# ntc-ai/sliders-conceptmod

Hardware: AMD Instinct MI355X
Metric: slider train-steps/sec (4-pass UNet fwd+bwd) (higher is better)
Workload: dtype fp16; 1 GPU; sdxl_1024_b2_r4; unet=sdxl, resolution=1024, per_gpu_batch=2, unet_batch=4, global_batch=2, lora_rank=4, train_method=noxattn, network_type=lierla, lora_params=2662400, scheduler=euler_a, parallelism=dp1, pre_roll=excluded, skip_dead_cfg_half=False, dedup_uncond=False, guidance_passes=1 batched UNet call (3 frozen + 1 adapted sub-batches)

## Files before the change

sliders_conceptmod_amd/csrc/gemm.hip:

```cpp
#include <cstdio>
#include <cstdlib>
#include <cstring>
#include <unordered_map>

#include "gemm_epilogue.h"
#include "gemm_tile.h"

#include <mutex>

namespace smi {

namespace {

constexpr int BM = 128, BN = 128, BK = 64;

struct ConvRow {
  int base;
  int oy, ox;
};

template <typename T, bool CONV>
__global__ __launch_bounds__(256) void gemm_nt_kernel(GemmParams p) {
  __shared__ __attribute__((aligned(16))) unsigned char smem[2 * BM * BK * 2];
  unsigned char* As = smem;
  unsigned char* Bs = smem + BM * BK * 2;

  const int tid = threadIdx.x;
  const int lane = tid & 63;
  const int wave = tid >> 6;
  const int wm = wave >> 1, wn = wave & 1;

  const int nbn = (p.N + BN - 1) / BN;
  const int wg = xcd_remap(blockIdx.x, gridDim.x);
  const int bm0 = (wg / nbn) * BM;
  const int bn0 = (wg % nbn) * BN;

  const uint32_t esz = 2;
  __amdgpu_buffer_rsrc_t rA, rW;
  if (CONV) {
    rA = make_rsrc(p.A, (uint32_t)((int64_t)p.Nb * p.Hin * p.Win * p.Cin * esz));
  } else {
    rA = make_rsrc(p.A, (uint32_t)(((int64_t)(p.M - 1) * p.lda + p.K) * esz));
  }
  rW = make_rsrc(p.W, (uint32_t)((int64_t)p.N * p.K * esz));

  const int sc = tid & 7;
  const int sr = tid >> 3;
  ConvRow crow[4];
  uint32_t a_rowoff[4];
  uint32_t w_rowoff[4];
#pragma unroll
  for (int i = 0; i < 4; ++i) {
    const int m = bm0 + sr + 32 * i;
    if (CONV) {
      if (m < p.M) {
        const int hw = p.Hout * p.Wout;
        const int img = m / hw;
        const int rem = m - img * hw;
        crow[i].base = img * p.Hin * p.Win;
        crow[i].oy = rem / p.Wout;
        crow[i].ox = rem - crow[i].oy * p.Wout;
      } else {
        crow[i].base = 0;
        crow[i].oy = -(1 << 20);
        crow[i].ox = -(1 << 20);
      }
      a_rowoff[i] = 0;
    } else {
      a_rowoff[i] = (m < p.M) ? (uint32_t)((int64_t)m * p.lda * esz) : OOB;
    }
    const int n = bn0 + sr + 32 * i;
    w_rowoff[i] = (n < p.N) ? (uint32_t)((int64_t)n * p.K * esz) : OOB;
  }

  u32x4 ra[4], rb[4];
  auto load_tile = [&](int kt) {
    const int k0 = kt * BK;
    const int kc = k0 + sc * 8;
    const bool kok = kc < p.K;
    if (CONV) {
      const int tap = k0 / p.Cin;
      const int c0 = k0 - tap * p.Cin;
      int ky, kx;
      conv_tap_yx(p, tap, ky, kx);
#pragma unroll
      for (int i = 0; i < 4; ++i) {
        int iy, ix;
        bool ok;
        if (p.transposed) {
          const int ty = crow[i].oy + 1 - ky, tx = crow[i].ox + 1 - kx;
          iy = ty / p.stride;
          ix = tx / p.stride;
          ok = (ty >= 0) && (tx >= 0) && (iy * p.stride == ty) && (ix * p.stride == tx) && (iy < p.Hin) &&
               (ix < p.Win);
        } else {
          iy = crow[i].oy * p.stride + ky + p.tap_oy;
          ix = crow[i].ox * p.stride + kx + p.tap_ox;
          if (p.upsample) {
            ok = (iy >= 0) && (ix >= 0) && (iy < 2 * p.Hin) && (ix < 2 * p.Win);
            iy >>= 1;
            ix >>= 1;
          } else {
            ok = (iy >= 0) && (ix >= 0) && (iy < p.Hin) && (ix < p.Win);
          }
        }
        const uint32_t off = ok ? (uint32_t)(((crow[i].base + iy * p.Win + ix) * (int64_t)p.Cin + c0 + sc * 8) * esz)
                                : OOB;
        ra[i] = buf_load16(rA, off);
      }
    } else {
#pragma unroll
      for (int i = 0; i < 4; ++i) {
        const uint32_t off = (kok && a_rowoff[i] != OOB) ? a_rowoff[i] + (uint32_t)kc * esz : OOB;
        ra[i] = buf_load16(rA, off);
      }
    }
#pragma unroll
    for (int i = 0; i < 4; ++i) {
      const uint32_t off = (kok && w_rowoff[i] != OOB) ? w_rowoff[i] + (uint32_t)kc * esz : OOB;
      rb[i] = buf_load16(rW, off);
    }
  };
  auto store_tile = [&]() {
#pragma unroll
    for (int i = 0; i < 4; ++i) {
      const int r = sr + 32 * i;
      const int off = r * 128 + ((sc ^ (r & 7)) << 4);
      *reinterpret_cast<u32x4*>(As + off) = ra[i];
      *reinterpret_cast<u32x4*>(Bs + off) = rb[i];
    }
  };

  f32x4 acc[4][4];
#pragma unroll
  for (int a = 0; a < 4; ++a)
#pragma unroll
    for (int b = 0; b < 4; ++b) acc[a][b] = f32x4{0.f, 0.f, 0.f, 0.f};

  const int nk = (p.K + BK - 1) / BK;
  const int fr = lane & 15;
  const int fq = lane >> 4;

  load_tile(0);
  for (int kt = 0; kt < nk; ++kt) {
    store_tile();
    __syncthreads();
    if (kt + 1 < nk) load_tile(kt + 1);
#pragma unroll
    for (int kk = 0; kk < 2; ++kk) {
      typename TT<T>::v8 xa[4], wb[4];
      const int ch = kk * 4 + fq;
#pragma unroll
      for (int i = 0; i < 4; ++i) {
        const int rm = wm * 64 + i * 16 + fr;
        Pack8<T> t;
        t.u = *reinterpret_cast<const u32x4*>(As + rm * 128 + ((ch ^ (rm & 7)) << 4));
        xa[i] = t.v;
        const int rn = wn * 64 + i * 16 + fr;
        Pack8<T> s;
        s.u = *reinterpret_cast<const u32x4*>(Bs + rn * 128 + ((ch ^ (rn & 7)) << 4));
        wb[i] = s.v;
      }
#pragma unroll
      for (int ni = 0; ni < 4; ++ni)
#pragma unroll
        for (int mi = 0; mi < 4; ++mi) acc[ni][mi] = TT<T>::mfma16(wb[ni], xa[mi], acc[ni][mi]);
    }
    __syncthreads();
  }

#pragma unroll
  for (int mi = 0; mi < 4; ++mi) {
    const int m = bm0 + wm * 64 + mi * 16 + fr;
    if (m >= p.M) continue;
    const bool lora_on = p.lora_r > 0 && m >= p.lora_row0;
    const int64_t vrow = p.rowvec ? epi_rowvec_offset(p, m) : 0;
#pragma unroll
    for (int ni = 0; ni < 4; ++ni) {
      const int n = bn0 + wn * 64 + ni * 16 + fq * 4;
      if (n >= p.N) continue;
      float v[4] = {acc[ni][mi][0], acc[ni][mi][1], acc[ni][mi][2], acc[ni][mi][3]};
      if (p.bias) epi_add<T, 4>(v, reinterpret_cast<const T*>(p.bias) + n);
      if (p.rowvec) epi_add<T, 4>(v, reinterpret_cast<const T*>(p.rowvec) + vrow + n);
      if (lora_on) epi_lora<4, false>(v, p, m, n);
      if (p.res) epi_add<T, 4>(v, reinterpret_cast<const T*>(p.res) + (int64_t)m * p.ldr + n);
      if (p.out_f32) epi_store_f32<4>(reinterpret_cast<float*>(p.C) + (int64_t)m * p.ldc + n, v);
      else epi_store<T, 4>(reinterpret_cast<T*>(p.C) + (int64_t)m * p.ldc + n, v);
    }
  }
}

template <typename T>
__global__ __launch_bounds__(256) void conv3x3_small_kernel(const T* __restrict__ in, const T* __restrict__ w,
                                                            const T* __restrict__ bias, void* out, int out_f32,
                                                            int Nb, int H, int W, int Cin, int Cout) {
  const int cg = (Cout + 3) / 4;
  const int64_t total = (int64_t)Nb * H * W * cg;
  for (int64_t idx = (int64_t)blockIdx.x * blockDim.x + threadIdx.x; idx < total;
       idx += (int64_t)gridDim.x * blockDim.x) {
    const int g = (int)(idx % cg);
    const int64_t pix = idx / cg;
    const int x = (int)(pix % W);
    const int y = (int)((pix / W) % H);
    const int n = (int)(pix / ((int64_t)W * H));
    const int co0 = g * 4;
    float acc[4] = {0.f, 0.f, 0.f, 0.f};
    for (int ky = 0; ky < 3; ++ky) {
      const int iy = y + ky - 1;
      if (iy < 0 || iy >= H) continue;
      for (int kx = 0; kx < 3; ++kx) {
        const int ix = x + kx - 1;
        if (ix < 0 || ix >= W) continue;
        const T* ip = in + (((int64_t)n * H + iy) * W + ix) * Cin;
        const int kb = (ky * 3 + kx) * Cin;
        for (int ci = 0; ci < Cin; ++ci) {
          const float v = to_f(ip[ci]);
#pragma unroll
          for (int j = 0; j < 4; ++j)
            if (co0 + j < Cout) acc[j] += v * to_f(w[(int64_t)(co0 + j) * 9 * Cin + kb + ci]);
        }
      }
    }
#pragma unroll
    for (int j = 0; j < 4; ++j) {
      if (co0 + j >= Cout) continue;
      float v = acc[j] + (bias ? to_f(bias[co0 + j]) : 0.f);
      if (out_f32)
        reinterpret_cast<float*>(out)[pix * Cout + co0 + j] = v;
      else
        reinterpret_cast<T*>(out)[pix * Cout + co0 + j] = from_f<T>(v);
    }
  }
}

template <typename T, int NS, int LR = 0>
__global__ __launch_bounds__(256) void splitk_finish_kernel(GemmParams p, const float* __restrict__ slab, int nsplit_rt) {
  const int nsplit = NS > 0 ? NS : nsplit_rt;
  const int n4 = p.N >> 2;
  const int64_t total = (int64_t)p.M * n4;
  const int64_t plane = (int64_t)p.M * p.N;
  for (int64_t idx = (int64_t)blockIdx.x * blockDim.x + threadIdx.x; idx < total; idx += (int64_t)gridDim.x * blockDim.x) {
    const int m = (int)(idx / n4);
    const int n = (int)(idx - (int64_t)m * n4) * 4;
    const float* sp = slab + (int64_t)m * p.N + n;
    f32x4 sum = *reinterpret_cast<const f32x4*>(sp);
    if constexpr (NS > 0) {
      f32x4 w[NS > 1 ? NS - 1 : 1];
#pragma unroll
      for (int s = 1; s < NS; ++s) w[s - 1] = *reinterpret_cast<const f32x4*>(sp + s * plane);
#pragma unroll
      for (int s = 1; s < NS; ++s)
#pragma unroll
        for (int j = 0; j < 4; ++j) sum[j] += w[s - 1][j];
    } else {
      for (int s = 1; s < nsplit; ++s) {
        const f32x4 w = *reinterpret_cast<const f32x4*>(sp + s * plane);
#pragma unroll
        for (int j = 0; j < 4; ++j) sum[j] += w[j];
      }
    }
    float v[4] = {sum[0], sum[1], sum[2], sum[3]};
    if (p.bias) epi_add<T, 4>(v, reinterpret_cast<const T*>(p.bias) + n);
    if (p.rowvec) epi_add<T, 4>(v, reinterpret_cast<const T*>(p.rowvec) + epi_rowvec_offset(p, m) + n);
    if (p.lora_r > 0 && m >= p.lora_row0) {
      if constexpr (LR > 0) epi_lora4_unrolled<LR>(v, p, m, n);
      else if (p.lora_r == 4) epi_lora4_unrolled<4>(v, p, m, n);
      else if (p.lora_r == 8) epi_lora4_unrolled<8>(v, p, m, n);
      else epi_lora<4, false>(v, p, m, n);
    }
    if (p.res) epi_add<T, 4>(v, reinterpret_cast<const T*>(p.res) + (int64_t)m * p.ldr + n);
    if (p.out_f32) epi_store_f32<4>(reinterpret_cast<float*>(p.C) + (int64_t)m * p.ldc + n, v);
    else epi_store<T, 4>(reinterpret_cast<T*>(p.C) + (int64_t)m * p.ldc + n, v);
  }
}

}

namespace {
struct TileName {
  GemmTile tile;
  const char* env;
  int code;
};
constexpr TileName kTileNames[] = {
    {GemmTile::Auto, nullptr, 0},
    {GemmTile::Auto, "no8ph", -1},
    {GemmTile::Auto, "no5ph", -1},
    {GemmTile::T128x128, nullptr, 13},
    {GemmTile::T128x128w8, "128", 1},
    {GemmTile::T128x128w8, nullptr, 5},
    {GemmTile::T256x128, "256", 2},
    {GemmTile::T64x128, "64", 14},
    {GemmTile::T64x128w4, "64w", 7},
    {GemmTile::T128x160, "160", 4},
    {GemmTile::T128x160w8, "160w", 10},
    {GemmTile::T128x160Deep, nullptr, 11},
    {GemmTile::T64x160, "64x160", 12},
    {GemmTile::Gemm3, "8ph", 100},
    {GemmTile::Gemm4, "5ph", 200},
    {GemmTile::V1, "v1", 300},
};
GemmTile tile_of_code(int code) {
  for (const TileName& t : kTileNames)
    if (t.code == code) return t.tile;
  return GemmTile::Auto;
}
int code_of_tile(GemmTile tile) {
  for (const TileName& t : kTileNames)
    if (t.tile == tile && t.code >= 0) return t.code;
  return 0;
}
const TileName* gemm_override() {
  static const TileName* o = []() -> const TileName* {
    const char* e = getenv("SMI_GEMM");
    for (const TileName& t : kTileNames)
      if (e && t.env && !strcmp(e, t.env)) return &t;
    return nullptr;
  }();
  return o;
}
bool forced_v1() { return gemm_override() && gemm_override()->tile == GemmTile::V1; }

GemmTile heuristic_tile(const GemmParams& p, bool gemm3) {
  if (gemm3 && !(p.conv && p.N % 256 != 0) && (int64_t)cdiv(p.M, 256) * cdiv(p.N, 256) >= 512 && gemm3_supported(p))
    return GemmTile::Gemm3;
  const bool rows256 = (int64_t)cdiv(p.M, 256) * cdiv(p.N, 128) >= 512 && (p.conv || p.N >= 4096);
  if (p.N % 160 == 0 && (!p.geglu_out || p.N % 320 == 0) && (int64_t)cdiv(p.M, 128) * cdiv(p.N, 128) >= 1024) {
    auto cost = [&](int bm, int bn, double eff) {
      const int64_t tiles = (int64_t)cdiv(p.M, bm) * cdiv(p.N, bn);
      return (double)((tiles + 255) / 256) * bm * bn / eff;
    };
    if (cost(128, 160, 1.04) < cost(rows256 ? 256 : 128, 128, rows256 ? 1.10 : 1.0)) return GemmTile::T128x160;
  }
  return rows256 ? GemmTile::T256x128 : GemmTile::T128x128w8;
}

GemmTile fit_tile(GemmTile tile, const GemmParams& p, bool gemm3) {
  switch (tile) {
    case GemmTile::Auto: return heuristic_tile(p, gemm3);
    case GemmTile::T64x128: return p.conv ? GemmTile::T128x128 : tile;
    case GemmTile::T128x160:
      return p.N % 8 == 0 && (!p.geglu_out || p.N % 320 == 0) ? tile : GemmTile::T128x128;
    case GemmTile::T64x160:
    case GemmTile::T128x160w8:
    case GemmTile::T128x160Deep: return p.N % 160 == 0 && !p.geglu_out ? tile : heuristic_tile(p, gemm3);
    case GemmTile::Gemm3: return gemm3_supported(p) ? tile : heuristic_tile(p, gemm3);
    case GemmTile::Gemm4: return gemm4_supported(p) ? tile : heuristic_tile(p, gemm3);
    default: return tile;
  }
}
int launch_tile(const GemmParams& p, GemmTile tile, hipStream_t stream) {
  if (tile == GemmTile::Gemm3) return launch_gemm3(p, stream);
  if (tile == GemmTile::Gemm4) return launch_gemm4(p, stream);
  if (tile == GemmTile::V1) return launch_v1(p, stream);
  return launch_gemm2(p, tile, stream);
}
}

bool gemm_geglu_supported(const GemmParams& p) { return !forced_v1() && gemm2_geglu_supported(p); }

namespace {
struct TuneKey {
  int v[18];
  bool operator==(const TuneKey& o) const { return memcmp(v, o.v, sizeof(v)) == 0; }
};
struct TuneHash {
  size_t operator()(const TuneKey& k) const {
    size_t h = 1469598103934665603ull;
    for (int x : k.v) h = (h ^ (size_t)(unsigned)x) * 1099511628211ull;
    return h;
  }
};
const char* tune_file() {
  static const char* f = getenv("SMI_TUNE_FILE");
  return (f && f[0]) ? f : nullptr;
}
std::unordered_map<TuneKey, int, TuneHash>& tune_cache() {
  static std::unordered_map<TuneKey, int, TuneHash> c;
  static bool loaded = false;
  if (!loaded) {
    loaded = true;
    if (const char* path = tune_file()) {
      if (FILE* fp = fopen(path, "r")) {
        for (;;) {
          TuneKey k;
          int choice = 0, got = 0;
          for (int i = 0; i < 18; ++i) got += fscanf(fp, "%d", &k.v[i]) == 1;
          got += fscanf(fp, "%d", &choice) == 1;
          if (got != 19) break;
          c[k] = choice;
        }
        fclose(fp);
      }
    }
  }
  return c;
}
void tune_persist(const TuneKey& k, int choice) {
  const char* path = tune_file();
  if (!path) return;
  if (FILE* fp = fopen(path, "a")) {
    for (int i = 0; i < 18; ++i) fprintf(fp, "%d ", k.v[i]);
    fprintf(fp, "%d\n", choice);
    fclose(fp);
  }
}
bool tune_enabled() {
  static int on = -1;
  if (on < 0) {
    const char* e = getenv("SMI_GEMM_TUNE");
    on = (e && !strcmp(e, "0")) ? 0 : 1;
  }
  return on == 1;
}
int launch_candidate(const GemmParams& p, GemmTile cand, hipStream_t stream) {
  return launch_tile(p, fit_tile(cand, p, true), stream);
}
GemmTile tuned_choice(const GemmParams& p, hipStream_t stream) {
  TuneKey key;
  const int taps = p.conv && (p.tap_w != 3 || p.tap_oy != -p.pad || p.tap_ox != -p.pad)
                       ? 16 * (p.tap_w * 64 + (p.tap_oy + 4) * 8 + (p.tap_ox + 4))
                       : 0;
  const int kv[18] = {(int)p.dtype, (int)p.conv, p.M, p.N, p.K, (int)(p.conv ? p.Cin : p.lda),
                      (int)(p.stride * 4 + p.upsample * 2 + p.transposed + taps), (int)(p.res != nullptr), p.lora_r,
                      (int)(p.geglu_out != nullptr), (int)p.out_f32, (int)(p.bias != nullptr),
                      (int)(p.rowvec != nullptr), (int)(p.conv ? p.Hin * 65536 + p.Win : p.ldc),
                      (int)(p.res ? p.ldr : 0), p.lora_seg, p.pad, (int)(p.res == p.C) + 2 * (int)(p.lora_r > 0 && p.up_sn == 1)};
  memcpy(key.v, kv, sizeof(kv));
  static std::mutex mu;
  std::lock_guard<std::mutex> lock(mu);
  auto& cache = tune_cache();
  auto it = cache.find(key);
  if (it != cache.end()) return tile_of_code(it->second);
  GemmTile cands[14];
  int nc = 0;
  cands[nc++] = GemmTile::Auto;
  const bool plain_conv = p.conv && p.stride == 1 && !p.upsample && !p.transposed;
  if (!p.conv || plain_conv) {
    cands[nc++] = GemmTile::T128x128w8;
    if ((int64_t)cdiv(p.M, 256) * cdiv(p.N, 128) >= 128) cands[nc++] = GemmTile::T256x128;
    if (p.N % 160 == 0 && (!p.geglu_out || p.N % 320 == 0)) cands[nc++] = GemmTile::T128x160;
    if (gemm3_supported(p) && (int64_t)cdiv(p.M, 256) * cdiv(p.N, 256) >= 192) cands[nc++] = GemmTile::Gemm3;
    if ((int64_t)cdiv(p.M, 128) * cdiv(p.N, 128) <= 512) cands[nc++] = GemmTile::T64x128w4;
    if (!p.geglu_out && p.N % 160 == 0 && (int64_t)cdiv(p.M, 128) * (p.N / 160) <= 256) cands[nc++] = GemmTile::T64x160;
    if (!p.geglu_out && p.N % 160 == 0 && p.K >= 1280 && (int64_t)cdiv(p.M, 128) * (p.N / 160) <= 128)
      cands[nc++] = GemmTile::T128x160Deep;
    if (gemm4_supported(p) && (int64_t)(p.M / 256) * (p.N / 320) >= 128) cands[nc++] = GemmTile::Gemm4;
    if (!p.geglu_out && p.N % 160 == 0 && p.N % 8 == 0 && (int64_t)cdiv(p.M, 128) * (p.N / 160) <= 512)
      cands[nc++] = GemmTile::T128x160w8;
  } else if (p.conv && p.upsample && gemm4_supported(p) && (int64_t)(p.M / 256) * (p.N / 320) >= 128) {
    cands[nc++] = GemmTile::Gemm4;
  }
  GemmTile best = GemmTile::Auto;
  if (nc > 1) {
    GemmParams q = p;
    void* tmp = nullptr;
    if (q.res == q.C) {
      const size_t bytes = ((size_t)(p.M - 1) * p.ldc + p.N) * (p.out_f32 ? 4 : 2);
      if (hipMalloc(&tmp, bytes) != hipSuccess) {
        (void)hipGetLastError();
        cache[key] = 0;
        return GemmTile::Auto;
      }
      q.C = tmp;
    }
    hipEvent_t a, b;
    if (hipEventCreate(&a) != hipSuccess || hipEventCreate(&b) != hipSuccess) {
      (void)hipGetLastError();
      if (tmp) (void)hipFree(tmp);
      cache[key] = 0;
      return GemmTile::Auto;
    }
    float tbest = 0.f, t0 = 0.f;
    static const bool dump = getenv("SMI_TUNE_DUMP") != nullptr;
    if (dump) fprintf(stderr, "[smi tune]");
    for (int i = 0; i < nc; ++i) {
      if (launch_candidate(q, cands[i], stream) != 0) continue;
      (void)hipEventRecord(a, stream);
      (void)launch_candidate(q, cands[i], stream);
      (void)launch_candidate(q, cands[i], stream);
      (void)hipEventRecord(b, stream);
      if (hipEventSynchronize(b) != hipSuccess) break;
      float ms = 0.f;
      (void)hipEventElapsedTime(&ms, a, b);
      if (dump) fprintf(stderr, " %d:%.1fus", code_of_tile(cands[i]), ms * 500.f);
      if (i == 0) { t0 = tbest = ms; continue; }
      if (ms < 0.97f * t0 && ms < tbest) { tbest = ms; best = cands[i]; }
    }
    if (dump)
      fprintf(stderr, "  -> %d   [%s M=%d N=%d K=%d%s%s%s%s]\n", code_of_tile(best), p.conv ? "conv" : "gemm", p.M, p.N, p.K,
              p.bias ? " bias" : "", p.res ? " res" : "", p.lora_r ? " lora" : "", p.geglu_out ? " geglu" : "");
    (void)hipEventDestroy(a);
    (void)hipEventDestroy(b);
    if (tmp) {
      (void)hipStreamSynchronize(stream);
      (void)hipFree(tmp);
    }
    (void)hipGetLastError();
  }
  cache[key] = code_of_tile(best);
  tune_persist(key, code_of_tile(best));
  return best;
}
}

namespace {
thread_local void* t_scratch = nullptr;
thread_local size_t t_scratch_bytes = 0;
int splitk_slices(const GemmParams& p) {
  static const bool on = []() { const char* e = getenv("SMI_GEMM_SPLITK"); return !(e && !strcmp(e, "0")); }();
  if (!on || !t_scratch || p.geglu_out || p.ksplit || !gemm2_supported(p) || p.N % 4 != 0) return 1;
  const int64_t tiles = (int64_t)cdiv(p.M, 128) * cdiv(p.N, 128);
  const int nk = cdiv(p.K, 64);
  static const int max_tiles = []() { const char* e = getenv("SMI_SPLITK_MAXTILES"); return e ? atoi(e) : 256; }();
  if (tiles > max_tiles || nk < 16) return 1;
  static const int few_tiles = []() { const char* e = getenv("SMI_SPLITK_FEWTILES"); return e ? atoi(e) : 95; }();
  static const int long_k = []() { const char* e = getenv("SMI_SPLITK_LONGK"); return e ? atoi(e) : 32; }();
  if (nk < long_k && tiles > few_tiles) return 1;
  int64_t lim = 16;
  const int64_t budget = 512;
  if (nk / 4 < lim) lim = nk / 4;
  const int64_t fit = (int64_t)(t_scratch_bytes / ((size_t)p.M * p.N * sizeof(float)));
  if (fit < lim) lim = fit;
  const int64_t tiles64 = (int64_t)cdiv(p.M, 64) * cdiv(p.N, 128);
  int64_t s = budget / tiles64 < lim ? budget / tiles64 : lim;
  if (s < 2) s = budget / tiles < lim ? budget / tiles : lim;
  return s < 1 ? 1 : (int)s;
}
int launch_splitk(const GemmParams& p, int S, GemmTile slice, hipStream_t stream) {
  SMI_CHECK(p.lora_seg % 4 == 0, "gemm: lora_seg %% 4 != 0");
  GemmParams q = p;
  q.C = t_scratch;
  q.ldc = p.N;
  q.out_f32 = 1;
  q.bias = q.res = q.rowvec = nullptr;
  q.lora_r = 0;
  q.lora_xa = q.lora_up = nullptr;
  q.ksplit = S;
  if (slice == GemmTile::Auto)
    slice = (int64_t)cdiv(p.M, 64) * cdiv(p.N, 128) * S <= 512 ? GemmTile::T64x128w4 : GemmTile::T128x128w8;
  if (launch_gemm2(q, slice, stream) != 0) return -1;
  const int64_t total = (int64_t)p.M * (p.N / 4);
  const int grid = (int)((total + 255) / 256 < 2048 ? (total + 255) / 256 : 2048);
#define FIN_R(TT_, NS_, LR_) hipLaunchKernelGGL((splitk_finish_kernel<TT_, NS_, LR_>), dim3(grid), dim3(256), 0, stream, p, (const float*)t_scratch, S)
#define FIN(TT_, NS_)                                                                                           \
  do {                                                                                                          \
    if (p.lora_r == 12) FIN_R(TT_, NS_, 12);                                                                    \
    else if (p.lora_r == 24) FIN_R(TT_, NS_, 24);                                                               \
    else FIN_R(TT_, NS_, 0);                                                                                    \
  } while (0)
#define FIN_T(TT_)                                                                                              \
  do {                                                                                                          \
    switch (S) {                                                                                                \
      case 2: FIN(TT_, 2); break;   case 3: FIN(TT_, 3); break;   case 4: FIN(TT_, 4); break;                   \
      case 5: FIN(TT_, 5); break;   case 6: FIN(TT_, 6); break;   case 7: FIN(TT_, 7); break;                   \
      case 8: FIN(TT_, 8); break;   case 9: FIN(TT_, 9); break;   case 10: FIN(TT_, 10); break;                 \
      case 11: FIN(TT_, 11); break; case 12: FIN(TT_, 12); break; case 13: FIN(TT_, 13); break;                 \
      case 14: FIN(TT_, 14); break; case 15: FIN(TT_, 15); break; case 16: FIN(TT_, 16); break;                 \
      default: FIN(TT_, 0);                                                                                     \
    }                                                                                                           \
  } while (0)
  if (p.dtype == DT_F16) FIN_T(f16); else FIN_T(bf16);
#undef FIN_T
#undef FIN
#undef FIN_R
  SMI_HIP(hipGetLastError());
  return 0;
}
}

namespace {
int g_upconv_phase_sel = -1;
}
void set_upconv_phase(int on) { g_upconv_phase_sel = on; }
bool upconv_phase_on() {
  static const bool env_on = []() { const char* e = getenv("SMI_UPCONV_PHASE"); return !(e && !strcmp(e, "0")); }();
  return g_upconv_phase_sel < 0 ? env_on : g_upconv_phase_sel != 0;
}
bool upconv_phase_takes(int lowres_pixels) {
  if (!upconv_phase_on()) return false;
  if (g_upconv_phase_sel > 0) return true;
  static const int floor_px = []() { const char* e = getenv("SMI_UPCONV_PHASE_MIN_PIXELS"); return e ? atoi(e) : 1024; }();
  return lowres_pixels >= floor_px;
}

void set_gemm_scratch(void* ws, size_t bytes) {
  t_scratch = ws;
  t_scratch_bytes = ws ? bytes : 0;
}

int launch_gemm(const GemmParams& p, hipStream_t stream) {
  SMI_CHECK(p.M > 0 && p.N > 0 && p.K > 0, "gemm: bad shape M=%d N=%d K=%d", p.M, p.N, p.K);
  SMI_CHECK(!p.geglu_out || gemm_geglu_supported(p), "gemm: fused GEGLU not available for this shape/layout");
  if (p.conv) {
    SMI_CHECK(p.K == p.tap_w * p.tap_w * p.Cin && p.M == p.Nb * p.Hout * p.Wout && (p.stride == 1 || p.stride == 2),
              "conv: inconsistent geometry");
    SMI_CHECK(p.tap_w == 3 || (p.tap_w == 2 && p.stride == 1 && !p.upsample && !p.transposed),
              "conv: a %d-wide tap grid (2 takes a plain stride-1 conv only)", p.tap_w);
  }
  static const bool splitk_debug = getenv("SMI_SPLITK_DEBUG") != nullptr;
  if (splitk_debug && gemm2_supported(p) && !p.geglu_out) {
    const char* es = getenv("SMI_SPLITK_S");
    const char* ev = getenv("SMI_SPLITK_V");
    const int S = es ? atoi(es) : 0;
    const GemmTile t = fit_tile(tile_of_code(ev ? atoi(ev) : 0), p, false);
    if (S > 1 && t_scratch && (size_t)S * p.M * p.N * sizeof(float) <= t_scratch_bytes) return launch_splitk(p, S, t, stream);
    if (S == 1) return launch_gemm2(p, t, stream);
  }
  const TileName* forced = gemm_override();
  if (!forced_v1()) {
    const int S = splitk_slices(p);
    if (S > 1) return launch_splitk(p, S, GemmTile::Auto, stream);
  }
  if (forced_v1() || !gemm2_supported(p)) return launch_v1(p, stream);
  if (forced) return launch_tile(p, fit_tile(forced->tile, p, false), stream);
  static int deep = -1, deep_k = 1280, small_grid = 128;
  if (deep < 0) {
    const char* e = getenv("SMI_GEMM_DEEP");
    deep = (e && !strcmp(e, "0")) ? 0 : 1;
    if (const char* k = getenv("SMI_GEMM_DEEP_K")) deep_k = atoi(k);
    if (const char* k = getenv("SMI_GEMM_SMALL_GRID")) small_grid = atoi(k);
  }
  const int64_t tiles160 = (int64_t)cdiv(p.M, 128) * (p.N / 160);
  if (deep && !p.geglu_out && p.N % 160 == 0 && p.K >= deep_k && tiles160 <= 320 && tiles160 > small_grid &&
      (!p.conv || (p.stride == 1 && !p.upsample && !p.transposed)))
    return launch_gemm2(p, GemmTile::T128x160Deep, stream);
  if (tune_enabled() && (int64_t)p.M * p.N >= (1 << 17)) return launch_candidate(p, tuned_choice(p, stream), stream);
  return launch_tile(p, heuristic_tile(p, true), stream);
}

int launch_gemm_on_tile(const GemmParams& p, int tile_code, int ksplit, int* ran_code, hipStream_t stream) {
  SMI_CHECK(p.M > 0 && p.N > 0 && p.K > 0, "gemm: bad shape M=%d N=%d K=%d", p.M, p.N, p.K);
  if (ran_code) *ran_code = 0;
  if (tile_code == 0 && ksplit <= 1) return launch_gemm(p, stream);
  GemmTile tile = tile_of_code(tile_code);
  SMI_CHECK(tile_code == 0 || tile != GemmTile::Auto, "gemm: unknown tile code %d", tile_code);
  SMI_CHECK(!p.geglu_out || gemm2_geglu_supported(p), "gemm: fused GEGLU not available for this shape/layout");
  tile = (tile == GemmTile::V1 || !gemm2_supported(p)) ? GemmTile::V1 : fit_tile(tile, p, false);
  if (ran_code) *ran_code = code_of_tile(tile);
  if (ksplit > 1) {
    SMI_CHECK(tile != GemmTile::V1 && tile != GemmTile::Gemm3 && tile != GemmTile::Gemm4 && !p.geglu_out && p.N % 4 == 0,
              "gemm: split-K takes a gemm2 tile as its slice kernel (tile code %d)", tile_code);
    SMI_CHECK(t_scratch && (size_t)ksplit * p.M * p.N * sizeof(float) <= t_scratch_bytes,
              "gemm: %d slices need a scratch of %zu bytes", ksplit, (size_t)ksplit * p.M * p.N * sizeof(float));
    return launch_splitk(p, ksplit, tile, stream);
  }
  return launch_tile(p, tile, stream);
}

int launch_v1(const GemmParams& p, hipStream_t stream) {
  SMI_CHECK(p.K % 8 == 0 && p.N % 4 == 0, "gemm: K %% 8 and N %% 4 must be 0 (K=%d N=%d)", p.K, p.N);
  SMI_CHECK(p.ldc % 4 == 0, "gemm: ldc %% 4 != 0");
  SMI_CHECK(p.lora_seg % 4 == 0, "gemm: lora_seg %% 4 != 0");
  SMI_CHECK(p.res == nullptr || p.ldr % 4 == 0, "gemm: ldr %% 4 != 0");
  if (p.conv) {
    SMI_CHECK(p.Cin % 64 == 0 && p.K == p.tap_w * p.tap_w * p.Cin, "conv: Cin %% 64 != 0 or K != taps*Cin (Cin=%d K=%d)",
              p.Cin, p.K);
    SMI_CHECK(p.M == p.Nb * p.Hout * p.Wout, "conv: M != Nb*Hout*Wout");
    SMI_CHECK((int64_t)p.Nb * p.Hin * p.Win * p.Cin * 2 < 0xFFFFFFF0ll, "conv: input larger than 4 GiB");
    SMI_CHECK(p.stride == 1 || p.stride == 2, "conv: stride");
  } else {
    SMI_CHECK(p.lda % 8 == 0, "gemm: lda %% 8 != 0");
    SMI_CHECK(((int64_t)(p.M - 1) * p.lda + p.K) * 2 < 0xFFFFFFF0ll, "gemm: A larger than 4 GiB");
  }
  SMI_CHECK((int64_t)p.N * p.K * 2 < 0xFFFFFFF0ll, "gemm: W larger than 4 GiB");
  const int grid = cdiv(p.M, BM) * cdiv(p.N, BN);
  if (p.dtype == DT_F16) {
    if (p.conv)
      hipLaunchKernelGGL((gemm_nt_kernel<f16, true>), dim3(grid), dim3(256), 0, stream, p);
    else
      hipLaunchKernelGGL((gemm_nt_kernel<f16, false>), dim3(grid), dim3(256), 0, stream, p);
  } else {
    if (p.conv)
      hipLaunchKernelGGL((gemm_nt_kernel<bf16, true>), dim3(grid), dim3(256), 0, stream, p);
    else
      hipLaunchKernelGGL((gemm_nt_kernel<bf16, false>), dim3(grid), dim3(256), 0, stream, p);
  }
  SMI_HIP(hipGetLastError());
  return 0;
}

int launch_conv3x3_small(int dtype, const void* in, const void* w, const void* bias, void* out, int out_f32, int Nb,
                         int H, int W, int Cin, int Cout, hipStream_t stream) {
  const int64_t total = (int64_t)Nb * H * W * ((Cout + 3) / 4);
  const int grid = (int)((total + 255) / 256 < 8192 ? (total + 255) / 256 : 8192);
  if (dtype == DT_F16)
    hipLaunchKernelGGL(conv3x3_small_kernel<f16>, dim3(grid), dim3(256), 0, stream, (const f16*)in, (const f16*)w,
                       (const f16*)bias, out, out_f32, Nb, H, W, Cin, Cout);
  else
    hipLaunchKernelGGL(conv3x3_small_kernel<bf16>, dim3(grid), dim3(256), 0, stream, (const bf16*)in,
                       (const bf16*)w, (const bf16*)bias, out, out_f32, Nb, H, W, Cin, Cout);
  SMI_HIP(hipGetLastError());
  return 0;
}

}
```

sliders_conceptmod_amd/csrc/gemm4.hip:

```cpp
#include "gemm_epilogue.h"
#include "gemm_tile.h"

namespace smi {
namespace {

constexpr int BM = 256, BN = 320, BK = 64;
constexpr int UNIT = 64 * BK * 2;
constexpr int ABYTES = 4 * UNIT;
constexpr int KBUF = ABYTES + 5 * UNIT;
constexpr int SMEM4 = 2 * KBUF;

template <typename T, int MODE>
__global__ __launch_bounds__(512) void gemm_5ph_kernel(GemmParams p) {
  constexpr bool CONV = MODE == 1 || MODE == 4;
  constexpr int TW = MODE == 4 ? 2 : 3;
  const int toy = MODE == 4 ? p.tap_oy : -1, tox = MODE == 4 ? p.tap_ox : -1;
  constexpr bool GEGLU = MODE == 2;
  constexpr bool UPS = MODE == 3;
  typedef typename TT<T>::v8 v8;
  extern __shared__ __attribute__((aligned(1024))) unsigned char smem[];

  const int tid = threadIdx.x;
  const int lane = tid & 63;
  const int wave = __builtin_amdgcn_readfirstlane(tid >> 6);
  const int wr = wave >> 1, wc = wave & 1, grp = wave >> 2;

  const int nbn = p.N / BN, nbm = p.M / BM;
  const int ntiles = nbn * nbm;
  const int nk = p.K / BK;
  const int G = gridDim.x;

  const int GW = raster_band(nbn);
  auto tile_origin = [&](int v, int& bm0, int& bn0) {
    int tm, tn;
    grouped_raster(xcd_remap(v, ntiles), nbm, nbn, GW, tm, tn);
    bm0 = __builtin_amdgcn_readfirstlane(tm * BM);
    bn0 = __builtin_amdgcn_readfirstlane(tn * BN);
  };

  const int lrow = lane >> 3, lslot = lane & 7;
  const int r64 = wave * 8 + lrow;
  const int chunk = lslot ^ lrow;
  const bool mix = !CONV && !UPS && p.lora_r > 0 && p.lora_row0 > 0 && 4 * (int64_t)p.lora_row0 == 3 * (int64_t)p.M;
  const int lda = (CONV || UPS) ? p.Cin : (int)p.lda;
  const bool arow = mix && wave >= 6;
  const uint32_t voffA = (uint32_t)(arow ? r64 - 48 : r64) * (uint32_t)(lda * 2) + chunk * 16;
  constexpr bool geglu = GEGLU;
  const int nhalf = p.N >> 1;
  const uint32_t voffB =
      (geglu ? (uint32_t)(((r64 >> 4) & 1) * nhalf + (r64 >> 5) * 80 + (r64 & 15))
             : (uint32_t)((r64 >> 5) * 160 + 8 * ((r64 & 15) >> 2) + 4 * ((r64 >> 4) & 1) + (r64 & 3))) *
          (uint32_t)(p.K * 2) +
      chunk * 16;
  const int64_t a_unit = (int64_t)(mix ? (arow ? 16 : 48) : 64) * lda * 2;
  const int64_t w_unit = (int64_t)(geglu ? 16 : 32) * p.K * 2;
  const int ldsw = wave * 1024;

  int bm0, bn0, bm1 = 0, bn1 = 0;
  int v = blockIdx.x;
  tile_origin(v, bm0, bn0);
  auto a_row0 = [&](int bm) { return mix ? (arow ? p.lora_row0 + (bm >> 2) : 3 * (bm >> 2)) : bm; };
  const char* a_cur = reinterpret_cast<const char*>(p.A) + (int64_t)a_row0(bm0) * lda * 2;
  const char* w_cur = reinterpret_cast<const char*>(p.W) + (int64_t)(geglu ? bn0 >> 1 : bn0) * p.K * 2;
  const char* a_nxt = a_cur;
  const char* w_nxt = w_cur;
  bool has_next = false;

  int am_cur[4] = {0, 0, 0, 0}, am_nxt[4] = {0, 0, 0, 0};
  auto conv_masks = [&](int bm, int (&am)[4]) {
    const int hw = p.Hin * p.Win;
#pragma unroll
    for (int u = 0; u < 4; ++u) {
      const int m = bm + u * 64 + r64;
      const int img = m / hw;
      const int rem = m - img * hw;
      const int oy = rem / p.Win, ox = rem - oy * p.Win;
      int mk = 0;
#pragma unroll
      for (int ky = 0; ky < TW; ++ky)
#pragma unroll
        for (int kx = 0; kx < TW; ++kx) {
          const bool ok = (unsigned)(oy + ky + toy) < (unsigned)p.Hin && (unsigned)(ox + kx + tox) < (unsigned)p.Win;
          mk |= ok ? (1 << (TW * ky + kx)) : 0;
        }
      am[u] = mk;
    }
  };
  if (CONV) conv_masks(bm0, am_cur);
  const int cpt = (CONV || UPS) ? p.Cin / BK : 1;
  const int cpt_magic = 65536 / cpt + 1;

  int ub_cur[4] = {0, 0, 0, 0}, uy_cur[4] = {0, 0, 0, 0}, ux_cur[4] = {0, 0, 0, 0};
  int ub_nxt[4] = {0, 0, 0, 0}, uy_nxt[4] = {0, 0, 0, 0}, ux_nxt[4] = {0, 0, 0, 0};
  auto ups_units = [&](int bm, int (&ub)[4], int (&uy)[4], int (&ux)[4]) {
    const int hw = p.Hout * p.Wout;
#pragma unroll
    for (int u = 0; u < 4; ++u) {
      const int m0 = bm + u * 64;
      const int img = m0 / hw;
      const int rem = m0 - img * hw;
      const int oy = rem / p.Wout;
      ub[u] = __builtin_amdgcn_readfirstlane(img * p.Hin * p.Win);
      uy[u] = __builtin_amdgcn_readfirstlane(oy);
      ux[u] = __builtin_amdgcn_readfirstlane(rem - oy * p.Wout);
    }
  };
  int voffU[3] = {0, 0, 0};
  if (UPS) {
    ups_units(bm0, ub_cur, uy_cur, ux_cur);
#pragma unroll
    for (int kx = 0; kx < 3; ++kx) voffU[kx] = ((r64 + kx - 1) >> 1) * (p.Cin * 2) + chunk * 16;
  }

  auto stage_a = [&](int u, int tp, unsigned char* buf) {
    const bool nx = tp >= nk;
    const int tt = nx ? tp - nk : tp;
    if (UPS) {
      const int tap = (tt * cpt_magic) >> 16;
      const int ky = (tap * 11) >> 5, kx = tap - 3 * ky;
      const int oy = nx ? uy_nxt[u] : uy_cur[u], ox0 = nx ? ux_nxt[u] : ux_cur[u], ub = nx ? ub_nxt[u] : ub_cur[u];
      const int iy2 = oy + ky - 1;
      const bool vok = (unsigned)iy2 < (unsigned)(2 * p.Hin);
      const char* base = reinterpret_cast<const char*>(p.A) +
                         ((int64_t)(ub + (iy2 >> 1) * p.Win + (ox0 >> 1)) * p.Cin + (tt - tap * cpt) * BK) * 2;
      const int vo = kx == 0 ? voffU[0] : (kx == 1 ? voffU[1] : voffU[2]);
      const bool ok = vok && (unsigned)(ox0 + r64 + kx - 1) < (unsigned)(2 * p.Win);
      glds16(ok ? (const void*)(base + vo) : (const void*)g_zero_page, buf + u * UNIT + ldsw);
    } else if (CONV) {
      const int tap = (tt * cpt_magic) >> 16;
      const int ky = TW == 2 ? tap >> 1 : (tap * 11) >> 5, kx = tap - TW * ky;
      const int64_t toff = ((int64_t)((ky + toy) * p.Win + (kx + tox)) * p.Cin + (tt - tap * cpt) * BK) * 2;
      const int mk = nx ? am_nxt[u] : am_cur[u];
      const char* src = (nx ? a_nxt : a_cur) + u * a_unit + toff + voffA;
      glds16(((mk >> tap) & 1) ? (const void*)src : (const void*)g_zero_page, buf + u * UNIT + ldsw);
    } else {
      const char* base = (nx ? a_nxt : a_cur) + (int64_t)tt * (BK * 2);
      glds16(base + u * a_unit + voffA, buf + u * UNIT + ldsw);
    }
  };
  auto stage_b = [&](int u, int tp, unsigned char* buf) {
    const char* base = tp < nk ? w_cur + (int64_t)tp * (BK * 2) : w_nxt + (int64_t)(tp - nk) * (BK * 2);
    glds16(base + u * w_unit + voffB, buf + ABYTES + u * UNIT + ldsw);
  };

  f32x4 acc[10][4];
#pragma unroll
  for (int a = 0; a < 10; ++a)
#pragma unroll
    for (int b = 0; b < 4; ++b) acc[a][b] = f32x4{0.f, 0.f, 0.f, 0.f};

  const int fr = lane & 15, fq = lane >> 4;
  const int swz0 = (fq ^ (fr & 7)) << 4;
  const int aoff0 = (wr * 64 + fr) * 128 + swz0, aoff1 = aoff0 ^ 64;
  const int boff0 = ABYTES + (wc * 32 + fr) * 128 + swz0, boff1 = boff0 ^ 64;

  v8 xa[2][4], wb[2][2];
  auto rdA = [&](const unsigned char* buf) {
#pragma unroll
    for (int i = 0; i < 4; ++i) {
      Pack8<T> t0, t1;
      t0.u = *reinterpret_cast<const u32x4*>(buf + aoff0 + i * 2048);
      t1.u = *reinterpret_cast<const u32x4*>(buf + aoff1 + i * 2048);
      xa[0][i] = t0.v;
      xa[1][i] = t1.v;
    }
  };
  auto rdB = [&](const unsigned char* buf, int u) {
#pragma unroll
    for (int i = 0; i < 2; ++i) {
      Pack8<T> t0, t1;
      t0.u = *reinterpret_cast<const u32x4*>(buf + boff0 + u * UNIT + i * 2048);
      t1.u = *reinterpret_cast<const u32x4*>(buf + boff1 + u * UNIT + i * 2048);
      wb[0][i] = t0.v;
      wb[1][i] = t1.v;
    }
  };
#define SMI_MMA5(U)                                                                                   \
  do {                                                                                                \
    __builtin_amdgcn_s_setprio(1);                                                                    \
    _Pragma("unroll") for (int kk = 0; kk < 2; ++kk) _Pragma("unroll") for (int ni = 0; ni < 2; ++ni) \
        _Pragma("unroll") for (int mi = 0; mi < 4; ++mi) acc[2 * (U) + ni][mi] =                      \
            TT<T>::mfma16(wb[kk][ni], xa[kk][mi], acc[2 * (U) + ni][mi]);                             \
    __builtin_amdgcn_s_setprio(0);                                                                    \
  } while (0)

  {
    unsigned char* b0 = smem;
    unsigned char* b1 = smem + KBUF;
#pragma unroll
    for (int u = 0; u < 4; ++u) stage_a(u, 0, b0);
#pragma unroll
    for (int u = 0; u < 5; ++u) stage_b(u, 0, b0);
#pragma unroll
    for (int u = 0; u < 3; ++u) {
      stage_b(u, 1, b1);
      stage_a(u, 1, b1);
    }
    asm volatile("s_waitcnt vmcnt(6)" ::: "memory");
    __builtin_amdgcn_s_barrier();
    if (grp == 1) __builtin_amdgcn_s_barrier();
  }

  unsigned gk = 0;
  while (true) {
    {
      const int vn = v + G;
      has_next = vn < ntiles;
      if (has_next) {
        tile_origin(vn, bm1, bn1);
        a_nxt = reinterpret_cast<const char*>(p.A) + (int64_t)a_row0(bm1) * lda * 2;
        if (CONV) conv_masks(bm1, am_nxt);
        if (UPS) ups_units(bm1, ub_nxt, uy_nxt, ux_nxt);
        w_nxt = reinterpret_cast<const char*>(p.W) + (int64_t)(geglu ? bn1 >> 1 : bn1) * p.K * 2;
      }
    }
    for (int t = 0; t < nk; ++t, ++gk) {
      unsigned char* cur = smem + (gk & 1) * KBUF;
      unsigned char* oth = smem + ((gk & 1) ^ 1) * KBUF;
      const bool s1 = t + 1 < nk || has_next;
      const bool s2 = t + 2 < nk || has_next;
      SMI_FENCE();
      rdB(cur, 0);
      SMI_FENCE();
      rdA(cur);
      SMI_FENCE();
      if (s1) {
        stage_b(3, t + 1, oth);
        stage_a(3, t + 1, oth);
      }
      SMI_FENCE();
      __builtin_amdgcn_s_barrier();
      asm volatile("s_waitcnt lgkmcnt(0)" ::: "memory");
      SMI_FENCE();
      SMI_MMA5(0);
      SMI_FENCE();
      __builtin_amdgcn_s_barrier();
      SMI_FENCE();
      rdB(cur, 1);
      SMI_FENCE();
      if (s1) stage_b(4, t + 1, oth);
      SMI_FENCE();
      __builtin_amdgcn_s_barrier();
      asm volatile("s_waitcnt lgkmcnt(0)" ::: "memory");
      SMI_FENCE();
      SMI_MMA5(1);
      SMI_FENCE();
      __builtin_amdgcn_s_barrier();
      SMI_FENCE();
      rdB(cur, 2);
      SMI_FENCE();
      if (s2) {
        stage_b(0, t + 2, cur);
        stage_a(0, t + 2, cur);
      }
      SMI_FENCE();
      __builtin_amdgcn_s_barrier();
      asm volatile("s_waitcnt lgkmcnt(0)" ::: "memory");
      SMI_FENCE();
      SMI_MMA5(2);
      SMI_FENCE();
      __builtin_amdgcn_s_barrier();
      SMI_FENCE();
      rdB(cur, 3);
      SMI_FENCE();
      if (s2) {
        stage_b(1, t + 2, cur);
        stage_a(1, t + 2, cur);
      }
      SMI_FENCE();
      __builtin_amdgcn_s_barrier();
      asm volatile("s_waitcnt lgkmcnt(0)" ::: "memory");
      SMI_FENCE();
      SMI_MMA5(3);
      SMI_FENCE();
      __builtin_amdgcn_s_barrier();
      SMI_FENCE();
      rdB(cur, 4);
      SMI_FENCE();
      if (s2) {
        stage_b(2, t + 2, cur);
        stage_a(2, t + 2, cur);
        asm volatile("s_waitcnt vmcnt(6)" ::: "memory");
      } else {
        asm volatile("s_waitcnt vmcnt(0)" ::: "memory");
      }
      SMI_FENCE();
      __builtin_amdgcn_s_barrier();
      asm volatile("s_waitcnt lgkmcnt(0)" ::: "memory");
      SMI_FENCE();
      SMI_MMA5(4);
      SMI_FENCE();
      __builtin_amdgcn_s_barrier();
    }
    if (grp == 0) __builtin_amdgcn_s_barrier();
    SMI_FENCE();

    const int rowf = mix ? 3 * (bm0 >> 2) + wr * 48 + fr : bm0 + wr * 64 + fr;
    const int rowa = mix ? p.lora_row0 + (bm0 >> 2) + wr * 16 + fr : bm0 + wr * 64 + 48 + fr;
    auto row_of = [&](int mi) { return mi < 3 ? rowf + mi * 16 : rowa; };
    const bool lora_tile = p.lora_r > 0 && (mix || bm0 + BM > p.lora_row0);
    const bool lora_mfma = epi_lora_mfma_form(p, BN) == EPI_MFMA_FWD;
    const int nblk = p.lora_r >> 2;
    const int xoff_t = p.lora_seg ? (bn0 / p.lora_seg) * p.lora_r : 0;
    auto epilogue_pair = [&](auto Uc) {
      constexpr int u = decltype(Uc)::value;
      const int n = bn0 + wc * 160 + u * 32 + fq * 8;
      float bv[8];
#pragma unroll
      for (int j = 0; j < 8; ++j) bv[j] = 0.f;
      if (p.bias) epi_unpack<T, 8>(bv, reinterpret_cast<const T*>(p.bias) + n);
      float au[2][4];
#pragma unroll
      for (int nip = 0; nip < 2; ++nip)
#pragma unroll
        for (int b = 0; b < 4; ++b) au[nip][b] = 0.f;
      if (lora_tile && lora_mfma) {
        const int ncol = bn0 + wc * 160 + u * 32;
#pragma unroll
        for (int nip = 0; nip < 2; ++nip)
#pragma unroll
          for (int b = 0; b < 4; ++b)
            if (b < nblk) au[nip][b] = epi_mfma_up(p, true, ncol + epi_pair_col(fr, nip), b, fq);
      }
      constexpr bool RES_AHEAD = !CONV;
      Pack8<T> rbuf[4];
      if (RES_AHEAD && p.res) {
#pragma unroll
        for (int mi = 0; mi < 4; ++mi)
          rbuf[mi] = epi_load<T, 8>(reinterpret_cast<const T*>(p.res) + (int64_t)row_of(mi) * p.ldr + n);
      }
#pragma unroll
      for (int mi = 0; mi < 4; ++mi) {
        const int m = row_of(mi);
        float vv[8];
#pragma unroll
        for (int j = 0; j < 4; ++j) {
          vv[j] = acc[2 * u][mi][j];
          vv[4 + j] = acc[2 * u + 1][mi][j];
          acc[2 * u][mi][j] = 0.f;
          acc[2 * u + 1][mi][j] = 0.f;
        }
        if (p.bias) epi_add<8>(vv, bv);
        if (p.rowvec) epi_add<T, 8>(vv, reinterpret_cast<const T*>(p.rowvec) + epi_rowvec_offset(p, m) + n);
        if (lora_tile && (!mix || mi == 3)) {
          const bool on = m >= p.lora_row0;
          if (lora_mfma) {
            f32x4 d0 = f32x4{0.f, 0.f, 0.f, 0.f}, d1 = d0;
            const float* xr = epi_mfma_xa(p, m, on, xoff_t, fq);
#pragma unroll
            for (int b = 0; b < 4; ++b)
              if (b < nblk) {
                const float bx = on ? xr[4 * b] : 0.f;
                d0 = epi_mfma_block(au[0][b], bx, d0);
                d1 = epi_mfma_block(au[1][b], bx, d1);
              }
            if (on) {
              epi_add_delta(vv, d0, p.lora_scale);
              epi_add_delta(vv + 4, d1, p.lora_scale);
            }
          } else if (on) {
            int nq = n;
            asm volatile("" : "+v"(nq));
            epi_lora<8, true, false>(vv, p, m, nq);
          }
        }
        if (p.res) {
          if constexpr (!RES_AHEAD) rbuf[mi] = epi_load<T, 8>(reinterpret_cast<const T*>(p.res) + (int64_t)m * p.ldr + n);
          epi_add<T, 8>(vv, rbuf[mi]);
        }
        if (p.out_f32) epi_store_f32<8>(reinterpret_cast<float*>(p.C) + (int64_t)m * p.ldc + n, vv);
        else epi_store<T, 8>(reinterpret_cast<T*>(p.C) + (int64_t)m * p.ldc + n, vv);
      }
    };
    auto epilogue_geglu = [&](auto Uc) {
      constexpr int u = decltype(Uc)::value;
      const int hc = (bn0 >> 1) + wc * 80 + u * 16 + fq * 4;
      float bh[4] = {0.f, 0.f, 0.f, 0.f}, bg[4] = {0.f, 0.f, 0.f, 0.f};
      if (p.bias) {
        Pack4<T> b0, b1;
        b0.u = *reinterpret_cast<const u32x2*>(reinterpret_cast<const T*>(p.bias) + hc);
        b1.u = *reinterpret_cast<const u32x2*>(reinterpret_cast<const T*>(p.bias) + nhalf + hc);
#pragma unroll
        for (int j = 0; j < 4; ++j) {
          bh[j] = to_f(b0.e[j]);
          bg[j] = to_f(b1.e[j]);
        }
      }
      T* gout = reinterpret_cast<T*>(p.geglu_out);
#pragma unroll
      for (int mi = 0; mi < 4; ++mi) {
        const int m = bm0 + wr * 64 + mi * 16 + fr;
        Pack4<T> h, g, o;
#pragma unroll
        for (int j = 0; j < 4; ++j) {
          float vh = acc[2 * u][mi][j], vg = acc[2 * u + 1][mi][j];
          acc[2 * u][mi][j] = 0.f;
          acc[2 * u + 1][mi][j] = 0.f;
          if (p.bias) {
            vh += bh[j];
            vg += bg[j];
          }
          h.e[j] = from_f<T>(vh);
          g.e[j] = from_f<T>(vg);
          o.e[j] = geglu_gate<T>(h.e[j], g.e[j]);
        }
        *reinterpret_cast<u32x2*>(gout + (int64_t)m * nhalf + hc) = o.u;
        if (m >= p.geglu_row0) {
          T* cp = reinterpret_cast<T*>(p.C) + (int64_t)m * p.ldc;
          *reinterpret_cast<u32x2*>(cp + hc) = h.u;
          *reinterpret_cast<u32x2*>(cp + nhalf + hc) = g.u;
        }
      }
    };
    if constexpr (GEGLU) {
      epilogue_geglu(std::integral_constant<int, 0>{});
      epilogue_geglu(std::integral_constant<int, 1>{});
      epilogue_geglu(std::integral_constant<int, 2>{});
      epilogue_geglu(std::integral_constant<int, 3>{});
      epilogue_geglu(std::integral_constant<int, 4>{});
    } else {
      epilogue_pair(std::integral_constant<int, 0>{});
      epilogue_pair(std::integral_constant<int, 1>{});
      epilogue_pair(std::integral_constant<int, 2>{});
      epilogue_pair(std::integral_constant<int, 3>{});
      epilogue_pair(std::integral_constant<int, 4>{});
    }
    SMI_FENCE();
    if (!has_next) break;
    if (grp == 1) __builtin_amdgcn_s_barrier();
    v += G;
    bm0 = bm1;
    bn0 = bn1;
    a_cur = a_nxt;
    w_cur = w_nxt;
    if (CONV) {
#pragma unroll
      for (int u = 0; u < 4; ++u) am_cur[u] = am_nxt[u];
    }
    if (UPS) {
#pragma unroll
      for (int u = 0; u < 4; ++u) {
        ub_cur[u] = ub_nxt[u];
        uy_cur[u] = uy_nxt[u];
        ux_cur[u] = ux_nxt[u];
      }
    }
  }
}

int device_cu_count() {
  static std::mutex mu;
  static int cus[64] = {0};
  int dev = 0;
  if (hipGetDevice(&dev) != hipSuccess || dev < 0 || dev >= 64) return 256;
  std::lock_guard<std::mutex> lock(mu);
  if (cus[dev] <= 0 &&
      (hipDeviceGetAttribute(&cus[dev], hipDeviceAttributeMultiprocessorCount, dev) != hipSuccess || cus[dev] <= 0))
    cus[dev] = 256;
  return cus[dev];
}

template <typename T, int MODE>
int launch_t(const GemmParams& p, hipStream_t stream) {
  static DynLdsOnce once;
  if (int rc = once.set((const void*)gemm_5ph_kernel<T, MODE>, SMEM4)) return rc;
  const int ncu = device_cu_count();
  const int ntiles = (p.M / BM) * (p.N / BN);
  const int grid = ntiles < ncu ? ntiles : ncu;
  hipLaunchKernelGGL((gemm_5ph_kernel<T, MODE>), dim3(grid), dim3(512), SMEM4, stream, p);
  SMI_HIP(hipGetLastError());
  return 0;
}

}

bool gemm4_supported(const GemmParams& p) {
  if (!gemm2_supported(p)) return false;
  if (p.geglu_out && (p.conv || p.out_f32 || p.res || p.rowvec || p.lora_r > 0 ||
                      (reinterpret_cast<uintptr_t>(p.geglu_out) & 15) != 0))
    return false;
  if (p.conv && (p.stride != 1 || p.pad != 1 || p.transposed || p.Cin % BK != 0 || p.K != p.tap_w * p.tap_w * p.Cin ||
                 p.M != p.Nb * p.Hout * p.Wout))
    return false;
  if (p.conv && p.tap_w != 3 && (p.tap_w != 2 || p.upsample)) return false;
  if (p.conv && p.upsample && (p.tap_oy != -1 || p.tap_ox != -1)) return false;
  if (p.conv && !p.upsample && (p.Hout != p.Hin || p.Wout != p.Win)) return false;
  if (p.conv && p.upsample && (p.Hout != 2 * p.Hin || p.Wout != 2 * p.Win || p.Wout % 64 != 0)) return false;
  if (p.M % BM != 0 || p.N % BN != 0 || p.K % BK != 0 || p.K < 2 * BK) return false;
  if (p.lora_seg % 8 != 0) return false;
  if (p.out_f32 && p.ldc % 4 != 0) return false;
  const int64_t lda = p.conv ? p.Cin : p.lda;
  if ((int64_t)BM * lda * 2 >= (1ll << 31) || (int64_t)BN * p.K * 2 >= (1ll << 31)) return false;
  return true;
}

int launch_gemm4(const GemmParams& p, hipStream_t stream) {
  const int mode = p.conv ? (p.upsample ? 3 : (p.tap_w == 2 ? 4 : 1)) : (p.geglu_out ? 2 : 0);
  if (p.dtype == DT_F16)
    return mode == 1   ? launch_t<f16, 1>(p, stream)
           : mode == 2 ? launch_t<f16, 2>(p, stream)
           : mode == 3 ? launch_t<f16, 3>(p, stream)
           : mode == 4 ? launch_t<f16, 4>(p, stream)
                       : launch_t<f16, 0>(p, stream);
  return mode == 1   ? launch_t<bf16, 1>(p, stream)
         : mode == 2 ? launch_t<bf16, 2>(p, stream)
         : mode == 3 ? launch_t<bf16, 3>(p, stream)
         : mode == 4 ? launch_t<bf16, 4>(p, stream)
                     : launch_t<bf16, 0>(p, stream);
}

}
```

Baseline: 6.711 steps/s.

## Interleave frozen/adapted rows and widen stores in GEGLU 5-phase GEMM

Extends the row-mixing tile layout (3 frozen + 1 adapted sub-batch rows per tile) to the GEGLU mode of the 256x320 GEMM, keyed on geglu_row0. This keeps the extra h/g stores for adapted rows spread evenly across tiles instead of concentrated in the last quarter. The weight staging for GEGLU is permuted so each lane's accumulator columns are contiguous, which lets the epilogue write 8-wide packed stores instead of 4-wide ones. The tuning cache key now encodes the GEGLU row split so tile choices are retuned for the new layout. The risk is extra index arithmetic, and any mismatch in the staging permutation would give wrong output.

```diff
diff --git a/sliders_conceptmod_amd/csrc/gemm.hip b/sliders_conceptmod_amd/csrc/gemm.hip
--- a/sliders_conceptmod_amd/csrc/gemm.hip
+++ b/sliders_conceptmod_amd/csrc/gemm.hip
@@ -421,9 +421,11 @@
   const int taps = p.conv && (p.tap_w != 3 || p.tap_oy != -p.pad || p.tap_ox != -p.pad)
                        ? 16 * (p.tap_w * 64 + (p.tap_oy + 4) * 8 + (p.tap_ox + 4))
                        : 0;
+  const bool geglu_q4 = 4 * (int64_t)p.geglu_row0 == 3 * (int64_t)p.M;
+  const int geglu_rows = !p.geglu_out ? 0 : p.geglu_row0 >= p.M ? 1 : p.geglu_row0 <= 0 ? 2 : geglu_q4 ? 3 : 4;
   const int kv[18] = {(int)p.dtype, (int)p.conv, p.M, p.N, p.K, (int)(p.conv ? p.Cin : p.lda),
                       (int)(p.stride * 4 + p.upsample * 2 + p.transposed + taps), (int)(p.res != nullptr), p.lora_r,
-                      (int)(p.geglu_out != nullptr), (int)p.out_f32, (int)(p.bias != nullptr),
+                      geglu_rows, (int)p.out_f32, (int)(p.bias != nullptr),
                       (int)(p.rowvec != nullptr), (int)(p.conv ? p.Hin * 65536 + p.Win : p.ldc),
                       (int)(p.res ? p.ldr : 0), p.lora_seg, p.pad, (int)(p.res == p.C) + 2 * (int)(p.lora_r > 0 && p.up_sn == 1)};
   memcpy(key.v, kv, sizeof(kv));
diff --git a/sliders_conceptmod_amd/csrc/gemm4.hip b/sliders_conceptmod_amd/csrc/gemm4.hip
--- a/sliders_conceptmod_amd/csrc/gemm4.hip
+++ b/sliders_conceptmod_amd/csrc/gemm4.hip
@@ -41,7 +41,9 @@
   const int lrow = lane >> 3, lslot = lane & 7;
   const int r64 = wave * 8 + lrow;
   const int chunk = lslot ^ lrow;
-  const bool mix = !CONV && !UPS && p.lora_r > 0 && p.lora_row0 > 0 && 4 * (int64_t)p.lora_row0 == 3 * (int64_t)p.M;
+  const int mix_row0 = GEGLU ? p.geglu_row0 : p.lora_row0;
+  const bool mix =
+      !CONV && !UPS && (GEGLU || p.lora_r > 0) && mix_row0 > 0 && 4 * (int64_t)mix_row0 == 3 * (int64_t)p.M;
   const int lda = (CONV || UPS) ? p.Cin : (int)p.lda;
   const bool arow = mix && wave >= 6;
   const uint32_t voffA = (uint32_t)(arow ? r64 - 48 : r64) * (uint32_t)(lda * 2) + chunk * 16;
@@ -52,14 +54,16 @@
              : (uint32_t)((r64 >> 5) * 160 + 8 * ((r64 & 15) >> 2) + 4 * ((r64 >> 4) & 1) + (r64 & 3))) *
           (uint32_t)(p.K * 2) +
       chunk * 16;
+  const uint32_t voffBw = geglu ? voffB + (uint32_t)(4 * ((r64 & 15) >> 2)) * (uint32_t)(p.K * 2) : voffB;
   const int64_t a_unit = (int64_t)(mix ? (arow ? 16 : 48) : 64) * lda * 2;
   const int64_t w_unit = (int64_t)(geglu ? 16 : 32) * p.K * 2;
+  const int64_t w_row4 = (int64_t)4 * p.K * 2;
   const int ldsw = wave * 1024;
 
   int bm0, bn0, bm1 = 0, bn1 = 0;
   int v = blockIdx.x;
   tile_origin(v, bm0, bn0);
-  auto a_row0 = [&](int bm) { return mix ? (arow ? p.lora_row0 + (bm >> 2) : 3 * (bm >> 2)) : bm; };
+  auto a_row0 = [&](int bm) { return mix ? (arow ? mix_row0 + (bm >> 2) : 3 * (bm >> 2)) : bm; };
   const char* a_cur = reinterpret_cast<const char*>(p.A) + (int64_t)a_row0(bm0) * lda * 2;
   const char* w_cur = reinterpret_cast<const char*>(p.W) + (int64_t)(geglu ? bn0 >> 1 : bn0) * p.K * 2;
   const char* a_nxt = a_cur;
@@ -140,7 +144,8 @@
   };
   auto stage_b = [&](int u, int tp, unsigned char* buf) {
     const char* base = tp < nk ? w_cur + (int64_t)tp * (BK * 2) : w_nxt + (int64_t)(tp - nk) * (BK * 2);
-    glds16(base + u * w_unit + voffB, buf + ABYTES + u * UNIT + ldsw);
+    if (geglu && u < 4) glds16(base + (8 * (u >> 1) + (u & 1)) * w_row4 + voffBw, buf + ABYTES + u * UNIT + ldsw);
+    else glds16(base + u * w_unit + voffB, buf + ABYTES + u * UNIT + ldsw);
   };
 
   f32x4 acc[10][4];
@@ -296,7 +301,7 @@
     SMI_FENCE();
 
     const int rowf = mix ? 3 * (bm0 >> 2) + wr * 48 + fr : bm0 + wr * 64 + fr;
-    const int rowa = mix ? p.lora_row0 + (bm0 >> 2) + wr * 16 + fr : bm0 + wr * 64 + 48 + fr;
+    const int rowa = mix ? mix_row0 + (bm0 >> 2) + wr * 16 + fr : bm0 + wr * 64 + 48 + fr;
     auto row_of = [&](int mi) { return mi < 3 ? rowf + mi * 16 : rowa; };
     const bool lora_tile = p.lora_r > 0 && (mix || bm0 + BM > p.lora_row0);
     const bool lora_mfma = epi_lora_mfma_form(p, BN) == EPI_MFMA_FWD;
@@ -372,52 +377,48 @@
         else epi_store<T, 8>(reinterpret_cast<T*>(p.C) + (int64_t)m * p.ldc + n, vv);
       }
     };
-    auto epilogue_geglu = [&](auto Uc) {
-      constexpr int u = decltype(Uc)::value;
-      const int hc = (bn0 >> 1) + wc * 80 + u * 16 + fq * 4;
-      float bh[4] = {0.f, 0.f, 0.f, 0.f}, bg[4] = {0.f, 0.f, 0.f, 0.f};
+    auto epilogue_geglu = [&](auto Uc, auto NUc) {
+      constexpr int u = decltype(Uc)::value, NU = decltype(NUc)::value, CW = 4 * NU;
+      const int hc = (bn0 >> 1) + wc * 80 + u * 16 + fq * CW;
+      float bh[CW], bg[CW];
+#pragma unroll
+      for (int j = 0; j < CW; ++j) bh[j] = bg[j] = 0.f;
       if (p.bias) {
-        Pack4<T> b0, b1;
-        b0.u = *reinterpret_cast<const u32x2*>(reinterpret_cast<const T*>(p.bias) + hc);
-        b1.u = *reinterpret_cast<const u32x2*>(reinterpret_cast<const T*>(p.bias) + nhalf + hc);
-#pragma unroll
-        for (int j = 0; j < 4; ++j) {
-          bh[j] = to_f(b0.e[j]);
-          bg[j] = to_f(b1.e[j]);
-        }
+        epi_unpack<T, CW>(bh, reinterpret_cast<const T*>(p.bias) + hc);
+        epi_unpack<T, CW>(bg, reinterpret_cast<const T*>(p.bias) + nhalf + hc);
       }
       T* gout = reinterpret_cast<T*>(p.geglu_out);
 #pragma unroll
       for (int mi = 0; mi < 4; ++mi) {
-        const int m = bm0 + wr * 64 + mi * 16 + fr;
-        Pack4<T> h, g, o;
-#pragma unroll
-        for (int j = 0; j < 4; ++j) {
-          float vh = acc[2 * u][mi][j], vg = acc[2 * u + 1][mi][j];
-          acc[2 * u][mi][j] = 0.f;
-          acc[2 * u + 1][mi][j] = 0.f;
-          if (p.bias) {
-            vh += bh[j];
-            vg += bg[j];
+        const int m = row_of(mi);
+        EpiPack<T, CW> h, g, o;
+#pragma unroll
+        for (int s = 0; s < NU; ++s)
+#pragma unroll
+          for (int j = 0; j < 4; ++j) {
+            float vh = acc[2 * (u + s)][mi][j], vg = acc[2 * (u + s) + 1][mi][j];
+            acc[2 * (u + s)][mi][j] = 0.f;
+            acc[2 * (u + s) + 1][mi][j] = 0.f;
+            if (p.bias) {
+              vh += bh[4 * s + j];
+              vg += bg[4 * s + j];
+            }
+            h.e[4 * s + j] = from_f<T>(vh);
+            g.e[4 * s + j] = from_f<T>(vg);
+            o.e[4 * s + j] = geglu_gate<T>(h.e[4 * s + j], g.e[4 * s + j]);
           }
-          h.e[j] = from_f<T>(vh);
-          g.e[j] = from_f<T>(vg);
-          o.e[j] = geglu_gate<T>(h.e[j], g.e[j]);
-        }
-        *reinterpret_cast<u32x2*>(gout + (int64_t)m * nhalf + hc) = o.u;
-        if (m >= p.geglu_row0) {
+        *reinterpret_cast<decltype(o.u)*>(gout + (int64_t)m * nhalf + hc) = o.u;
+        if (mix ? mi == 3 : m >= p.geglu_row0) {
           T* cp = reinterpret_cast<T*>(p.C) + (int64_t)m * p.ldc;
-          *reinterpret_cast<u32x2*>(cp + hc) = h.u;
-          *reinterpret_cast<u32x2*>(cp + nhalf + hc) = g.u;
+          *reinterpret_cast<decltype(h.u)*>(cp + hc) = h.u;
+          *reinterpret_cast<decltype(g.u)*>(cp + nhalf + hc) = g.u;
         }
       }
     };
     if constexpr (GEGLU) {
-      epilogue_geglu(std::integral_constant<int, 0>{});
-      epilogue_geglu(std::integral_constant<int, 1>{});
-      epilogue_geglu(std::integral_constant<int, 2>{});
-      epilogue_geglu(std::integral_constant<int, 3>{});
-      epilogue_geglu(std::integral_constant<int, 4>{});
+      epilogue_geglu(std::integral_constant<int, 0>{}, std::integral_constant<int, 2>{});
+      epilogue_geglu(std::integral_constant<int, 2>{}, std::integral_constant<int, 2>{});
+      epilogue_geglu(std::integral_constant<int, 4>{}, std::integral_constant<int, 1>{});
     } else {
       epilogue_pair(std::integral_constant<int, 0>{});
       epilogue_pair(std::integral_constant<int, 1>{});
```

New measurement: 6.701 steps/s. No clear change (-0.1%).
